# leggedrobotics/qed-splatter

Hardware: AMD Instinct MI355X
Metric: train iters/sec @ 1080p, 500k Gaussians (fwd + loss + bwd + Adam; camera-steps/s over all GPUs) (higher is better)
Workload: dtype f32

## Files before the change

### qed_splatter_amd/csrc/project.hip

```cpp
#include "qed_common.h"

namespace qed {

struct Cam {
    float R[9];
    float t[3];
    float fx, fy, cx, cy;
    float campos[3];
};

__device__ __forceinline__ Cam load_cam(const float* __restrict__ viewmats, const float* __restrict__ Ks, int c) {
    Cam cam;
    const float* V = viewmats + 16 * c;
    const float* K = Ks + 9 * c;
#pragma unroll
    for (int i = 0; i < 3; ++i) {
#pragma unroll
        for (int j = 0; j < 3; ++j) cam.R[3 * i + j] = V[4 * i + j];
        cam.t[i] = V[4 * i + 3];
    }
    cam.fx = K[0]; cam.fy = K[4]; cam.cx = K[2]; cam.cy = K[5];
#pragma unroll
    for (int j = 0; j < 3; ++j)
        cam.campos[j] = campos_component(cam.R[0 + j], cam.R[3 + j], cam.R[6 + j], cam.t[0], cam.t[1], cam.t[2]);
// ... 262 lines not shown
        float mx = 0.f, my = 0.f, z = 0.f, ca = 0.f, cb = 0.f, cc = 0.f, op = 0.f;
        float rgb[3] = {0.f, 0.f, 0.f};
        if (p.valid) {
            rad = (int)p.radius;
            mx = p.mx; my = p.my; z = p.z; ca = p.ca; cb = p.cb; cc = p.cc;
            op = op_raw;
            if (flags & QED_F_LOGIT_OPAC) op = sigmoidf_dev(op);
            if (flags & QED_F_ANTIALIASED) op *= p.comp;
            if (sh_degree >= 0) {
                const float dir[3] = {mean[0] - cam.campos[0], mean[1] - cam.campos[1], mean[2] - cam.campos[2]};
                float J[9];
                unsigned mask;
                sh_color_jac_dyn(sh_degree, sh0 + (size_t)n * sh0_stride, shN + (size_t)n * shN_stride, dir, rgb, J, mask);
                if (sh_jac != nullptr) {
#pragma unroll
                    for (int i = 0; i < 9; ++i) sh_jac[(size_t)i * total + slot] = J[i];
                    sh_jac[(size_t)9 * total + slot] = __uint_as_float(mask);
                }
            } else {
                const float* cptr = sh0 + (size_t)n * sh0_stride;
                rgb[0] = cptr[0]; rgb[1] = cptr[1]; rgb[2] = cptr[2];
                if (flags & QED_F_SIGMOID_COLORS) {
                    rgb[0] = sigmoidf_dev(rgb[0]); rgb[1] = sigmoidf_dev(rgb[1]); rgb[2] = sigmoidf_dev(rgb[2]);
                }
            }
            const float tau = logf(255.f * op);
            int x0, y0, x1, y1;
            if (flags & QED_F_TIGHT_TILES) tight_tile_rect(mx, my, p.radius, ca, cb, cc, tau, tile_w, tile_h, x0, y0, x1, y1);
            else tile_rect(mx, my, p.radius, tile_w, tile_h, x0, y0, x1, y1);
            ntiles = (x1 - x0) * (y1 - y0);
            m_c0 = make_float4(mx, my, ca, cb); m_cc = cc; m_tau = tau; m_rect = pack_tile_rect(x0, y0, x1);
            r0 = make_float4(mx, my, ca, cb);
            r1 = make_float4(cc, op, rgb[0], rgb[1]);
            r2 = make_float4(rgb[2], (flags & QED_F_DEPTH_CHANNEL) ? z : 0.f, tau,
                             __uint_as_float(pack_tile_rect(x0, y0, x1)));
        }
        radii[slot] = rad;
        means2d[2 * slot] = mx; means2d[2 * slot + 1] = my;
        depths[slot] = z;
        conics[3 * slot] = ca; conics[3 * slot + 1] = cb; conics[3 * slot + 2] = cc;
        opac_out[slot] = op;
        colors_out[3 * slot] = rgb[0]; colors_out[3 * slot + 1] = rgb[1]; colors_out[3 * slot + 2] = rgb[2];
        splats[3 * slot] = r0; splats[3 * slot + 1] = r1; splats[3 * slot + 2] = r2;
    }
    if (tile_masks != nullptr) {
        __shared__ __attribute__((aligned(16))) float4 s_c0[4][64];
        __shared__ __attribute__((aligned(16))) float4 s_c1[4][64];
        __shared__ unsigned s_rect[4][64];
        __shared__ int s_pref[4][65];
        __shared__ int s_nz[4][64];
        __shared__ unsigned long long s_start[4][64];
        __shared__ unsigned long long s_mask[4][64];
        const int lane = threadIdx.x & 63, wid = threadIdx.x >> 6;
        const int cand = ntiles <= 64 ? ntiles : 0;
        int x = cand;
#pragma unroll
        for (int o = 1; o < 64; o <<= 1) {
            const int y = __shfl_up(x, o, 64);
            if (lane >= o) x += y;
        }
        const int pref = x - cand;
        const int wtot = __shfl(x, 63, 64);
        const unsigned long long nz = __ballot(cand > 0);
        s_pref[wid][lane] = pref;
        s_c0[wid][lane] = make_float4(m_c0.x, m_c0.y, m_c0.w, m_tau);
        s_c1[wid][lane] = make_float4(0.5f * m_c0.z, 0.5f * m_cc, __builtin_amdgcn_rcpf(m_c0.z), __builtin_amdgcn_rcpf(m_cc));
        s_rect[wid][lane] = m_rect;
        s_mask[wid][lane] = 0ull;
        s_start[wid][lane] = 0ull;
        if (cand > 0) s_nz[wid][__popcll(nz & ((1ull << lane) - 1ull))] = lane;
        __builtin_amdgcn_fence(__ATOMIC_ACQ_REL, "wavefront");
        __builtin_amdgcn_wave_barrier();
        if (cand > 0) atomicOr(&s_start[wid][pref >> 6], 1ull << (pref & 63));
        __builtin_amdgcn_fence(__ATOMIC_ACQ_REL, "wavefront");
        __builtin_amdgcn_wave_barrier();
        int before = 0;
        for (int j0 = 0; j0 < wtot; j0 += 64) {
            const unsigned long long word = s_start[wid][j0 >> 6];
            const int j = j0 + lane;
            const int k = before + __popcll(word & ((2ull << lane) - 1ull)) - 1;
            before += __popcll(word);
            if (j >= wtot) continue;
            const int g = s_nz[wid][k];
            const int local = j - s_pref[wid][g];
            const float4 c0 = s_c0[wid][g], c1 = s_c1[wid][g];
            const unsigned r = s_rect[wid][g];
            const int w = (int)(r >> 22);
            const int row = (int)(((float)local + 0.5f) * __builtin_amdgcn_rcpf((float)w));
            const int tx = (int)(r & 2047u) + local - row * w, ty = (int)((r >> 11) & 2047u) + row;
            CullGauss cg;
            cg.b = c0.z; cg.ha = c1.x; cg.hc = c1.y; cg.ia = c1.z; cg.ic = c1.w;
            cg.X0 = (float)(tx * QED_TILE) + 0.5f - c0.x; cg.Y0 = (float)(ty * QED_TILE) + 0.5f - c0.y;
            const float ax = fmaxf(fabsf(cg.X0), fabsf(cg.X0 + 15.f)), ay = fmaxf(fabsf(cg.Y0), fabsf(cg.Y0 + 15.f));
            cg.thr = c0.w + 1e-3f + 8e-6f * (2.f * (cg.ha * ax * ax + cg.hc * ay * ay) + fabsf(cg.b) * ax * ay);
            if (tile_may_touch(cg)) atomicOr(&s_mask[wid][g], 1ull << local);
        }
        __builtin_amdgcn_fence(__ATOMIC_ACQ_REL, "wavefront");
        __builtin_amdgcn_wave_barrier();
        if (slot < total) {
            unsigned long long mask = ~0ull;
            if (cand > 0) { mask = s_mask[wid][lane]; ntiles = __popcll(mask); }
            reinterpret_cast<uint4*>(tile_masks)[slot] = make_uint4((unsigned)ntiles, m_rect, (unsigned)mask, (unsigned)(mask >> 32));
        }
    }
    if (slot < total) tiles_per_gauss[slot] = ntiles;
    __shared__ int wsum[4];
    const int v = wave_sum_i(ntiles);
    if ((threadIdx.x & 63) == 0) wsum[threadIdx.x >> 6] = v;
    __syncthreads();
    if (threadIdx.x == 0) block_sums[blockIdx.x] = wsum[0] + wsum[1] + wsum[2] + wsum[3];
}

template <int DEG>
__device__ __forceinline__ void sh_bwd(const float* __restrict__ sh0, const float* __restrict__ shN,
                                       const float* dir, const float* v_rgb_in, float* v_coef ,
                                       float* v_dir ) {
    constexpr int K = (DEG + 1) * (DEG + 1);
    const float n2 = dir[0] * dir[0] + dir[1] * dir[1] + dir[2] * dir[2];
    const float inorm = rsqrtf(n2);
    const float x = dir[0] * inorm, y = dir[1] * inorm, z = dir[2] * inorm;
    float b[K];
    sh_basis<DEG>(x, y, z, b);
    float c[3 * K];
    load_sh<K>(sh0, shN, c);
    float col[3] = {0.f, 0.f, 0.f};
#pragma unroll
    for (int k = 0; k < K; ++k) {
        col[0] += b[k] * c[3 * k]; col[1] += b[k] * c[3 * k + 1]; col[2] += b[k] * c[3 * k + 2];
    }
    float v[3];
#pragma unroll
    for (int ch = 0; ch < 3; ++ch) v[ch] = (col[ch] + 0.5f >= 0.f) ? v_rgb_in[ch] : 0.f;
#pragma unroll
    for (int k = 0; k < K; ++k) {
        v_coef[3 * k] += b[k] * v[0]; v_coef[3 * k + 1] += b[k] * v[1]; v_coef[3 * k + 2] += b[k] * v[2];
    }
    if constexpr (DEG > 0) {
        float bx[K], by[K], bz[K];
        sh_basis_grad<DEG>(x, y, z, bx, by, bz);
        float vx = 0.f, vy = 0.f, vz = 0.f;
#pragma unroll
        for (int k = 1; k < K; ++k) {
            const float w = c[3 * k] * v[0] + c[3 * k + 1] * v[1] + c[3 * k + 2] * v[2];
            vx += bx[k] * w; vy += by[k] * w; vz += bz[k] * w;
        }
        const float dot = vx * x + vy * y + vz * z;
        v_dir[0] += (vx - dot * x) * inorm;
        v_dir[1] += (vy - dot * y) * inorm;
        v_dir[2] += (vz - dot * z) * inorm;
    }
}

template <int DEG, bool STREAM>
__device__ __forceinline__ void sh_bwd_jac(const float* __restrict__ jac , size_t plane,
                                           const float* dir, const float* v_rgb_in, float* __restrict__ o0,
                                           float* __restrict__ oN, float* v_coef, float* v_dir , bool compact,
                                           float* stage_b = nullptr ,
                                           float* stage_v = nullptr) {
    constexpr int K = (DEG + 1) * (DEG + 1);
    float J[9];
#pragma unroll
    for (int i = 0; i < (DEG > 0 ? 9 : 0); ++i) J[i] = jac[(size_t)i * plane];
    const unsigned mask = __float_as_uint(jac[(size_t)9 * plane]);
    const float n2 = dir[0] * dir[0] + dir[1] * dir[1] + dir[2] * dir[2];
    const float inorm = rsqrtf(n2);
    const float x = dir[0] * inorm, y = dir[1] * inorm, z = dir[2] * inorm;
    float v[3];
#pragma unroll
    for (int ch = 0; ch < 3; ++ch) v[ch] = (mask >> ch & 1u) ? v_rgb_in[ch] : 0.f;
    if (STREAM && compact) {
        o0[0] = v[0]; o0[1] = v[1]; o0[2] = v[2];
    } else {
        float b[K];
        sh_basis<DEG>(x, y, z, b);
        if constexpr (STREAM) {
            o0[0] = b[0] * v[0]; o0[1] = b[0] * v[1]; o0[2] = b[0] * v[2];
            if (stage_b != nullptr) {
                constexpr int KS = (K + 3) & ~3;
#pragma unroll
                for (int k4 = 0; k4 < KS / 4; ++k4)
                    reinterpret_cast<float4*>(stage_b)[k4] =
                        make_float4(b[4 * k4], 4 * k4 + 1 < K ? b[4 * k4 + 1] : 0.f, 4 * k4 + 2 < K ? b[4 * k4 + 2] : 0.f,
                                    4 * k4 + 3 < K ? b[4 * k4 + 3] : 0.f);
                *reinterpret_cast<float4*>(stage_v) = make_float4(v[0], v[1], v[2], 0.f);
            } else {
#pragma unroll
                for (int k = 1; k < K; ++k) {
                    oN[3 * (k - 1)] = b[k] * v[0]; oN[3 * (k - 1) + 1] = b[k] * v[1]; oN[3 * (k - 1) + 2] = b[k] * v[2];
                }
            }
        } else {
#pragma unroll
            for (int k = 0; k < K; ++k) {
                v_coef[3 * k] += b[k] * v[0]; v_coef[3 * k + 1] += b[k] * v[1]; v_coef[3 * k + 2] += b[k] * v[2];
            }
        }
    }
    if constexpr (DEG > 0) {
        const float vx = J[0] * v[0] + J[1] * v[1] + J[2] * v[2];
        const float vy = J[3] * v[0] + J[4] * v[1] + J[5] * v[2];
        const float vz = J[6] * v[0] + J[7] * v[1] + J[8] * v[2];
        const float dot = vx * x + vy * y + vz * z;
        v_dir[0] += (vx - dot * x) * inorm;
        v_dir[1] += (vy - dot * y) * inorm;
        v_dir[2] += (vz - dot * z) * inorm;
    }
}

template <int DEG>
__device__ __forceinline__ void sh_bwd_stream(const float* __restrict__ sh0, const float* __restrict__ shN,
                                              const float* dir, const float* v_rgb_in, float* __restrict__ o0,
                                              float* __restrict__ oN, float* v_dir , bool compact) {
    constexpr int K = (DEG + 1) * (DEG + 1);
    const float n2 = dir[0] * dir[0] + dir[1] * dir[1] + dir[2] * dir[2];
    const float inorm = rsqrtf(n2);
    const float x = dir[0] * inorm, y = dir[1] * inorm, z = dir[2] * inorm;
    float b[K];
    sh_basis<DEG>(x, y, z, b);
    float col[3] = {0.f, 0.f, 0.f};
    float S[3][3] = {{0.f, 0.f, 0.f}, {0.f, 0.f, 0.f}, {0.f, 0.f, 0.f}};
    {
        float bx[K], by[K], bz[K];
        sh_basis_grad<DEG>(x, y, z, bx, by, bz);
#pragma unroll
        for (int k = 0; k < K; ++k) {
            const float* ck = k == 0 ? sh0 : shN + 3 * (k - 1);
#pragma unroll
            for (int ch = 0; ch < 3; ++ch) {
                const float c = ck[ch];
                col[ch] += b[k] * c;
                if (k > 0) { S[0][ch] += bx[k] * c; S[1][ch] += by[k] * c; S[2][ch] += bz[k] * c; }
            }
        }
    }
    float v[3];
#pragma unroll
    for (int ch = 0; ch < 3; ++ch) v[ch] = (col[ch] + 0.5f >= 0.f) ? v_rgb_in[ch] : 0.f;
    if (compact) {
        o0[0] = v[0]; o0[1] = v[1]; o0[2] = v[2];
    } else {
        o0[0] = b[0] * v[0]; o0[1] = b[0] * v[1]; o0[2] = b[0] * v[2];
#pragma unroll
        for (int k = 1; k < K; ++k) {
            oN[3 * (k - 1)] = b[k] * v[0]; oN[3 * (k - 1) + 1] = b[k] * v[1]; oN[3 * (k - 1) + 2] = b[k] * v[2];
        }
    }
    if constexpr (DEG > 0) {
        const float vx = S[0][0] * v[0] + S[0][1] * v[1] + S[0][2] * v[2];
        const float vy = S[1][0] * v[0] + S[1][1] * v[1] + S[1][2] * v[2];
        const float vz = S[2][0] * v[0] + S[2][1] * v[1] + S[2][2] * v[2];
        const float dot = vx * x + vy * y + vz * z;
        v_dir[0] += (vx - dot * x) * inorm;
        v_dir[1] += (vy - dot * y) * inorm;
        v_dir[2] += (vz - dot * z) * inorm;
    }
}

template <int K>
__device__ __forceinline__ void sh_grad_store_staged(const float* __restrict__ stage ,
                                                     int lane, float* __restrict__ out ,
                                                     int stride, int n_rows) {
    constexpr int KS = (K + 3) & ~3, FP = 3 * (K - 1);
    const float* sv = stage + 64 * KS;
    int g = lane / FP, j = lane - g * FP;
#pragma unroll 5
    for (int it = 0; it < FP; ++it) {
        const int k = (j * 171) >> 9;
        const int ch = j - 3 * k;
        if (g < n_rows) out[(size_t)g * stride + j] = stage[g * KS + k + 1] * sv[4 * g + ch];
        g += 64 / FP; j += 64 % FP;
        if (j >= FP) { j -= FP; ++g; }
    }
}

template <int DEG, bool ONE_CAM, bool JAC = false>
#ifndef QED_PBWD_WAVES
#define QED_PBWD_WAVES 2
#endif
__global__ void __launch_bounds__(256) __attribute__((amdgpu_waves_per_eu(QED_PBWD_WAVES, QED_PBWD_WAVES)))
project_bwd_kernel(int N, int C, const float* __restrict__ means, const float* __restrict__ quats,
                   const float* __restrict__ scales, const float* __restrict__ opacities,
                   const float* __restrict__ sh0, int sh0_stride, const float* __restrict__ shN, int shN_stride,
                   const float* __restrict__ viewmats, const float* __restrict__ Ks, int width, int height,
                   float eps2d, unsigned flags, const int* __restrict__ radii, const float4* __restrict__ vsplat,
                   float* __restrict__ v_means, float* __restrict__ v_quats, float* __restrict__ v_scales,
                   float* __restrict__ v_opacities, float* __restrict__ v_sh0, int v_sh0_stride,
                   float* __restrict__ v_shN, int v_shN_stride, float* __restrict__ v_viewmats,
                   const float* __restrict__ sh_jac) {
    constexpr int K = DEG < 0 ? 1 : (DEG + 1) * (DEG + 1);
    const int n = blockIdx.x * 256 + threadIdx.x;
    const bool active = n < N;

    float vm[3] = {0.f, 0.f, 0.f}, vq[4] = {0.f, 0.f, 0.f, 0.f}, vs[3] = {0.f, 0.f, 0.f}, vo = 0.f;
    constexpr bool kStreamSH = ONE_CAM && DEG >= 0;
    float vcoef[kStreamSH ? 1 : 3 * K];
#pragma unroll
    for (int i = 0; i < (kStreamSH ? 1 : 3 * K); ++i) vcoef[i] = 0.f;
    bool sh_written = false;
    constexpr bool kStageSH = JAC && kStreamSH && K > 1;
    constexpr int kKS = (K + 3) & ~3;
    constexpr int kStageFloats = kStageSH ? 64 * (kKS + 4) : 1;
    __shared__ __attribute__((aligned(16))) float s_stage[4 * kStageFloats];
    float* const stage_wave = s_stage + (threadIdx.x >> 6) * kStageFloats;
    const bool staged = kStageSH && !(flags & QED_F_SH_GRAD_COMPACT);
    float* const stage_b = staged ? stage_wave + (threadIdx.x & 63) * kKS : nullptr;
    float* const stage_v = staged ? stage_wave + 64 * kKS + 4 * (threadIdx.x & 63) : nullptr;

    float mean[3] = {0.f, 0.f, 0.f}, qraw[4] = {1.f, 0.f, 0.f, 0.f}, q[4], sraw[3] = {0.f, 0.f, 0.f}, s[3];
    float qin = 1.f, oraw = 0.f, oact = 0.f;
    if (active) {
        mean[0] = means[3 * n]; mean[1] = means[3 * n + 1]; mean[2] = means[3 * n + 2];
        qraw[0] = quats[4 * n]; qraw[1] = quats[4 * n + 1]; qraw[2] = quats[4 * n + 2]; qraw[3] = quats[4 * n + 3];
        sraw[0] = scales[3 * n]; sraw[1] = scales[3 * n + 1]; sraw[2] = scales[3 * n + 2];
        oraw = opacities[n];
    }
    qin = rsqrtf(qraw[0] * qraw[0] + qraw[1] * qraw[1] + qraw[2] * qraw[2] + qraw[3] * qraw[3]);
#pragma unroll
    for (int i = 0; i < 4; ++i) q[i] = qraw[i] * qin;
#pragma unroll
    for (int i = 0; i < 3; ++i) s[i] = (flags & QED_F_LOG_SCALES) ? __expf(sraw[i]) : sraw[i];
    oact = (flags & QED_F_LOGIT_OPAC) ? sigmoidf_dev(oraw) : oraw;

    for (int c = 0; c < C; ++c) {
        const Cam cam = load_cam(viewmats, Ks, c);
        const size_t slot = (size_t)c * N + n;
        const bool vis = active && radii[slot] > 0;
        float vR[9] = {0.f, 0.f, 0.f, 0.f, 0.f, 0.f, 0.f, 0.f, 0.f}, vt[3] = {0.f, 0.f, 0.f};
        if constexpr (kStageSH) {
            if (staged && !vis) {
#pragma unroll
                for (int k4 = 0; k4 < kKS / 4; ++k4) reinterpret_cast<float4*>(stage_b)[k4] = make_float4(0.f, 0.f, 0.f, 0.f);
                *reinterpret_cast<float4*>(stage_v) = make_float4(0.f, 0.f, 0.f, 0.f);
            }
        }
        if (vis) {
            Proj p;
            project_one(cam, mean, q, s, width, height, eps2d, -3.0e38f, 3.0e38f, -1.f, p);
            const float4 g0 = vsplat[4 * slot], g1 = vsplat[4 * slot + 1], g2 = vsplat[4 * slot + 2];
            const float v_mx = g0.x, v_my = g0.y;
            float v_ca = g1.x, v_cb = g1.y, v_cc = g1.z;
            const float v_op = g1.w;
            const float v_rgb[3] = {g2.x, g2.y, g2.z};
            const float v_depth = (flags & QED_F_DEPTH_CHANNEL) ? g2.w : 0.f;

            float v_comp = 0.f;
            if (flags & QED_F_ANTIALIASED) {
                vo += v_op * p.comp;
                v_comp = v_op * oact;
            } else {
                vo += v_op;
            }
            const float g01 = 0.5f * v_cb;
            const float bh = 0.5f * (p.A + p.Cc), hd = 0.5f * (p.A - p.Cc);
            const float rr = __builtin_amdgcn_sqrtf(hd * hd + p.B * p.B);
            const float lp = bh + rr, ilp = __builtin_amdgcn_rcpf(lp), lm = p.det * ilp, ilm = __builtin_amdgcn_rcpf(lm);
            float ux, uy;
            if (hd >= 0.f) { ux = hd + rr; uy = p.B; }
            else { ux = p.B; uy = rr - hd; }
            const float un = ux * ux + uy * uy;
            if (un > 0.f) { const float ir = __builtin_amdgcn_rsqf(un); ux *= ir; uy *= ir; } else { ux = 1.f; uy = 0.f; }
            const float wx = -uy, wy = ux;
            const float gux = v_ca * ux + g01 * uy, guy = g01 * ux + v_cc * uy;
            const float gwx = v_ca * wx + g01 * wy, gwy = g01 * wx + v_cc * wy;
            float hpp = -(ux * gux + uy * guy) * ilp * ilp;
            float hpm = -(ux * gwx + uy * gwy) * ilp * ilm;
            float hmm = -(wx * gwx + wy * gwy) * ilm * ilm;
            if (flags & QED_F_ANTIALIASED) {
                const float det_conic = 1.f / p.det;
                const float v_sqr = v_comp * 0.5f / (p.comp + 1e-6f);
                const float om = 1.f - p.comp * p.comp;
                hpp += v_sqr * (om * ilp - eps2d * det_conic);
                hmm += v_sqr * (om * ilm - eps2d * det_conic);
            }
            float vT[6];
#pragma unroll
            for (int j = 0; j < 3; ++j) {
                const float pu = ux * p.Tm[j] + uy * p.Tm[3 + j], pw = wx * p.Tm[j] + wy * p.Tm[3 + j];
                const float qu = hpp * pu + hpm * pw, qw = hpm * pu + hmm * pw;
                vT[j] = 2.f * (ux * qu + wx * qw);
                vT[3 + j] = 2.f * (uy * qu + wy * qw);
            }
            const float rz = p.rz, rz2 = rz * rz, rz3 = rz2 * rz;
            const float j00 = cam.fx * rz, j02 = -cam.fx * p.tx * rz2;
            const float j11 = cam.fy * rz, j12 = -cam.fy * p.ty * rz2;
            const float vJ00 = vT[0] * p.W[0] + vT[1] * p.W[1] + vT[2] * p.W[2];
            const float vJ02 = vT[0] * p.W[6] + vT[1] * p.W[7] + vT[2] * p.W[8];
            const float vJ11 = vT[3] * p.W[3] + vT[4] * p.W[4] + vT[5] * p.W[5];
            const float vJ12 = vT[3] * p.W[6] + vT[4] * p.W[7] + vT[5] * p.W[8];
            float vW[9];
#pragma unroll
            for (int j = 0; j < 3; ++j) {
                vW[j] = j00 * vT[j];
                vW[3 + j] = j11 * vT[3 + j];
                vW[6 + j] = j02 * vT[j] + j12 * vT[3 + j];
            }
            float vx = v_mx * cam.fx * rz;
            float vy = v_my * cam.fy * rz;
            float vz = -v_mx * cam.fx * p.x * rz2 - v_my * cam.fy * p.y * rz2 - vJ00 * cam.fx * rz2 -
                       vJ11 * cam.fy * rz2 + v_depth;
            if (!p.clamp_x) {
                vx += -cam.fx * rz2 * vJ02;
                vz += 2.f * cam.fx * p.tx * rz3 * vJ02;
            } else {
                vz += cam.fx * p.tx * rz3 * vJ02;
            }
            if (!p.clamp_y) {
                vy += -cam.fy * rz2 * vJ12;
                vz += 2.f * cam.fy * p.ty * rz3 * vJ12;
            } else {
                vz += cam.fy * p.ty * rz3 * vJ12;
            }
            float vmw[3];
#pragma unroll
            for (int j = 0; j < 3; ++j) vmw[j] = cam.R[j] * vx + cam.R[3 + j] * vy + cam.R[6 + j] * vz;
            float vM[9];
#pragma unroll
            for (int i = 0; i < 3; ++i)
#pragma unroll
                for (int j = 0; j < 3; ++j)
                    vM[3 * i + j] = cam.R[i] * vW[j] + cam.R[3 + i] * vW[3 + j] + cam.R[6 + i] * vW[6 + j];
            float vdir[3] = {0.f, 0.f, 0.f};
            if constexpr (DEG >= 0) {
                const float dir[3] = {mean[0] - cam.campos[0], mean[1] - cam.campos[1], mean[2] - cam.campos[2]};
                if constexpr (JAC) {
                    const size_t plane = (size_t)C * N;
                    sh_bwd_jac<(DEG < 0 ? 0 : DEG), kStreamSH>(sh_jac + slot, plane, dir, v_rgb,
                                                                v_sh0 + (size_t)n * v_sh0_stride,
                                                                v_shN + (size_t)n * v_shN_stride, vcoef, vdir,
                                                                (flags & QED_F_SH_GRAD_COMPACT) != 0, stage_b, stage_v);
                    sh_written = true;
                } else if constexpr (kStreamSH) {
                    sh_bwd_stream<(DEG < 0 ? 0 : DEG)>(sh0 + (size_t)n * sh0_stride, shN + (size_t)n * shN_stride, dir,
                                                       v_rgb, v_sh0 + (size_t)n * v_sh0_stride,
                                                       v_shN + (size_t)n * v_shN_stride, vdir,
                                                       (flags & QED_F_SH_GRAD_COMPACT) != 0);
                    sh_written = true;
                } else {
                    sh_bwd<(DEG < 0 ? 0 : DEG)>(sh0 + (size_t)n * sh0_stride, shN + (size_t)n * shN_stride, dir, v_rgb,
                                                vcoef, vdir);
                }
            } else {
                if (flags & QED_F_SIGMOID_COLORS) {
                    const float* cptr = sh0 + (size_t)n * sh0_stride;
#pragma unroll
                    for (int ch = 0; ch < 3; ++ch) {
                        const float sg = sigmoidf_dev(cptr[ch]);
                        vcoef[ch] += v_rgb[ch] * sg * (1.f - sg);
                    }
                } else {
                    vcoef[0] += v_rgb[0]; vcoef[1] += v_rgb[1]; vcoef[2] += v_rgb[2];
                }
            }
            vm[0] += vmw[0] + vdir[0]; vm[1] += vmw[1] + vdir[1]; vm[2] += vmw[2] + vdir[2];
            float vRq[9];
#pragma unroll
            for (int i = 0; i < 3; ++i)
#pragma unroll
                for (int j = 0; j < 3; ++j) {
                    vRq[3 * i + j] = vM[3 * i + j] * s[j];
                    vs[j] += vM[3 * i + j] * p.Rq[3 * i + j];
                }
            const float w = q[0], x = q[1], y = q[2], z = q[3];
            float vqn[4];
            vqn[0] = 2.f * (x * (vRq[7] - vRq[5]) + y * (vRq[2] - vRq[6]) + z * (vRq[3] - vRq[1]));
            vqn[1] = 2.f * (-2.f * x * (vRq[4] + vRq[8]) + y * (vRq[1] + vRq[3]) + z * (vRq[2] + vRq[6]) +
                            w * (vRq[7] - vRq[5]));
            vqn[2] = 2.f * (x * (vRq[1] + vRq[3]) - 2.f * y * (vRq[0] + vRq[8]) + z * (vRq[5] + vRq[7]) +
                            w * (vRq[2] - vRq[6]));
            vqn[3] = 2.f * (x * (vRq[2] + vRq[6]) + y * (vRq[5] + vRq[7]) - 2.f * z * (vRq[0] + vRq[4]) +
                            w * (vRq[3] - vRq[1]));
            vq[0] += vqn[0]; vq[1] += vqn[1]; vq[2] += vqn[2]; vq[3] += vqn[3];

            if (v_viewmats != nullptr) {
                const float vmc[3] = {vx, vy, vz};
#pragma unroll
                for (int i = 0; i < 3; ++i) {
#pragma unroll
                    for (int j = 0; j < 3; ++j) {
                        vR[3 * i + j] = vmc[i] * mean[j] + vW[3 * i] * p.M[3 * j] + vW[3 * i + 1] * p.M[3 * j + 1] +
                                        vW[3 * i + 2] * p.M[3 * j + 2];
                    }
                    vt[i] = vmc[i];
                }
#pragma unroll
                for (int i = 0; i < 3; ++i) {
                    const float rv = cam.R[3 * i] * vdir[0] + cam.R[3 * i + 1] * vdir[1] + cam.R[3 * i + 2] * vdir[2];
#pragma unroll
                    for (int j = 0; j < 3; ++j) vR[3 * i + j] += rv * cam.campos[j];
                    vt[i] += rv;
                }
            }
        }
        if constexpr (kStageSH) {
            if (staged) {
                __builtin_amdgcn_fence(__ATOMIC_RELEASE, "wavefront");
                __builtin_amdgcn_wave_barrier();
                __builtin_amdgcn_fence(__ATOMIC_ACQUIRE, "wavefront");
                const int n0 = blockIdx.x * 256 + (threadIdx.x & ~63);
                sh_grad_store_staged<K>(stage_wave, threadIdx.x & 63, v_shN + (size_t)n0 * v_shN_stride, v_shN_stride,
                                        N - n0);
            }
        }
        if (v_viewmats != nullptr) {
#pragma unroll
            for (int i = 0; i < 12; ++i) {
                float v = i < 9 ? vR[i] : vt[i - 9];
                v = wave_sum(v);
                if ((threadIdx.x & 63) == 0 && v != 0.f) {
                    const int row = i < 9 ? i / 3 : i - 9, col = i < 9 ? i % 3 : 3;
                    atomicAdd(&v_viewmats[16 * c + 4 * row + col], v);
                }
            }
        }
    }
    if (!active) return;
    const float dq = vq[0] * q[0] + vq[1] * q[1] + vq[2] * q[2] + vq[3] * q[3];
#pragma unroll
    for (int i = 0; i < 4; ++i) v_quats[4 * n + i] = (vq[i] - dq * q[i]) * qin;
#pragma unroll
    for (int i = 0; i < 3; ++i) {
        v_means[3 * n + i] = vm[i];
        v_scales[3 * n + i] = (flags & QED_F_LOG_SCALES) ? vs[i] * s[i] : vs[i];
    }
    v_opacities[n] = (flags & QED_F_LOGIT_OPAC) ? vo * oact * (1.f - oact) : vo;
    float* o0 = v_sh0 + (size_t)n * v_sh0_stride;
    if constexpr (kStreamSH) {
        if (!sh_written) {
            o0[0] = 0.f; o0[1] = 0.f; o0[2] = 0.f;
            if (K > 1 && !(flags & QED_F_SH_GRAD_COMPACT) && !staged) {
                float* oN = v_shN + (size_t)n * v_shN_stride;
#pragma unroll
                for (int i = 0; i < 3 * (K - 1); ++i) oN[i] = 0.f;
            }
        }
    } else {
        o0[0] = vcoef[0]; o0[1] = vcoef[1]; o0[2] = vcoef[2];
        if constexpr (K > 1) {
            float* oN = v_shN + (size_t)n * v_shN_stride;
#pragma unroll
            for (int i = 0; i < 3 * (K - 1); ++i) oN[i] = vcoef[3 + i];
        }
    }
}

template <int DEG>
__global__ void __launch_bounds__(256)
sh_grad_from_views_kernel(int N, int n_views, const float* __restrict__ means, const float* __restrict__ viewmats,
                          long long viewmat_stride, const float* __restrict__ v_views, long long view_stride,
                          float scale, float* __restrict__ v_sh0, int v_sh0_stride, float* __restrict__ v_shN,
                          int v_shN_stride) {
    constexpr int K = (DEG + 1) * (DEG + 1);
    const int n = blockIdx.x * 256 + threadIdx.x;
    if (n >= N) return;
    const float mean[3] = {means[3 * n], means[3 * n + 1], means[3 * n + 2]};
    float acc[3 * K];
#pragma unroll
    for (int i = 0; i < 3 * K; ++i) acc[i] = 0.f;
    for (int c = 0; c < n_views; ++c) {
        const float* vm = viewmats + viewmat_stride * c;
        const float* vv = v_views + view_stride * c + (size_t)n * 3;
        const float v[3] = {vv[0], vv[1], vv[2]};
        if (v[0] == 0.f && v[1] == 0.f && v[2] == 0.f) continue;
        float dir[3];
#pragma unroll
        for (int j = 0; j < 3; ++j)
            dir[j] = mean[j] - campos_component(vm[0 + j], vm[4 + j], vm[8 + j], vm[3], vm[7], vm[11]);
        const float inorm = rsqrtf(dir[0] * dir[0] + dir[1] * dir[1] + dir[2] * dir[2]);
        float b[K];
        sh_basis<DEG>(dir[0] * inorm, dir[1] * inorm, dir[2] * inorm, b);
#pragma unroll
        for (int k = 0; k < K; ++k) {
            acc[3 * k] += b[k] * v[0]; acc[3 * k + 1] += b[k] * v[1]; acc[3 * k + 2] += b[k] * v[2];
        }
    }
    float* o0 = v_sh0 + (size_t)n * v_sh0_stride;
    o0[0] = acc[0] * scale; o0[1] = acc[1] * scale; o0[2] = acc[2] * scale;
    if constexpr (K > 1) {
        float* oN = v_shN + (size_t)n * v_shN_stride;
#pragma unroll
        for (int i = 0; i < 3 * (K - 1); ++i) oN[i] = acc[3 + i] * scale;
    }
}

__global__ void camera_setup_kernel(int C, const float* __restrict__ c2w, const float* __restrict__ intr,
                                    float* __restrict__ viewmats, float* __restrict__ Ks) {
    const int c = blockIdx.x * blockDim.x + threadIdx.x;
    if (c >= C) return;
    const float* m = c2w + 12 * c;
    float R[9], t[3];
#pragma unroll
    for (int i = 0; i < 3; ++i) {
        R[3 * i] = m[4 * i];
        R[3 * i + 1] = -m[4 * i + 1];
        R[3 * i + 2] = -m[4 * i + 2];
        t[i] = m[4 * i + 3];
    }
    float* V = viewmats + 16 * c;
#pragma unroll
    for (int i = 0; i < 3; ++i) {
#pragma unroll
        for (int j = 0; j < 3; ++j) V[4 * i + j] = R[3 * j + i];
        V[4 * i + 3] = -(R[i] * t[0] + R[3 + i] * t[1] + R[6 + i] * t[2]);
    }
    V[12] = 0.f; V[13] = 0.f; V[14] = 0.f; V[15] = 1.f;
    float* K = Ks + 9 * c;
    K[0] = intr[4 * c]; K[1] = 0.f; K[2] = intr[4 * c + 2];
    K[3] = 0.f; K[4] = intr[4 * c + 1]; K[5] = intr[4 * c + 3];
    K[6] = 0.f; K[7] = 0.f; K[8] = 1.f;
}

}

using namespace qed;

extern "C" int qed_camera_setup(int32_t C, const float* c2w, const float* intrinsics, float* viewmats, float* Ks,
                                void* stream) {
    QED_REQUIRE(C >= 1 && c2w && intrinsics && viewmats && Ks, "bad arguments");
    hipLaunchKernelGGL(camera_setup_kernel, dim3((C + 63) / 64), dim3(64), 0, (hipStream_t)stream, C, c2w, intrinsics,
                       viewmats, Ks);
    return check_launch("qed_camera_setup");
}

extern "C" int qed_project_fwd(int32_t N, int32_t C, const float* means, const float* quats, const float* scales,
                               const float* opacities, const float* sh0, int32_t sh0_stride, const float* shN,
                               int32_t shN_stride, int32_t sh_degree, const float* viewmats, const float* Ks,
                               int32_t width, int32_t height, int32_t tile_w, int32_t tile_h, float eps2d,
                               float near_plane, float far_plane, float radius_clip, uint32_t flags, int32_t* radii,
                               float* means2d, float* depths, float* conics, float* opac_out, float* colors_out,
                               float* splats, int32_t* tiles_per_gauss, uint64_t* tile_masks, int32_t* block_sums,
                               float* viewmats_out, float* Ks_out, float* sh_jac, void* stream) {
    QED_REQUIRE(N >= 0 && C >= 1, "N >= 0 and C >= 1 required");
    QED_REQUIRE(sh_degree <= 3, "SH degree > 3 unsupported (reference config uses sh_degree = 3)");
    QED_REQUIRE(width > 0 && height > 0 && tile_w > 0 && tile_h > 0, "bad image / tile extents");
    QED_REQUIRE((long long)tile_w * tile_h < (1ll << 30), "too many tiles");
    if (N == 0) return QED_OK;
    QED_REQUIRE(means && quats && scales && opacities && sh0 && viewmats && Ks, "null input");
    QED_REQUIRE(sh_degree <= 0 || shN, "shN required for sh_degree > 0");
    QED_REQUIRE(radii && means2d && depths && conics && opac_out && colors_out && splats && tiles_per_gauss &&
                    block_sums, "null output");
    QED_REQUIRE(!(flags & QED_F_CAMERA_C2W) || (viewmats_out && Ks_out), "QED_F_CAMERA_C2W needs viewmats_out and Ks_out");
    QED_REQUIRE(tile_masks == nullptr || (flags & QED_F_TIGHT_TILES), "tile_masks goes with QED_F_TIGHT_TILES");
    QED_REQUIRE(((uintptr_t)tile_masks & 15) == 0, "tile_masks must be 16-byte aligned");
    const long long total = (long long)C * N;
    const unsigned grid = (unsigned)((total + 255) / 256);
#define QED_LAUNCH_PF(ONE)                                                                                           \
    hipLaunchKernelGGL(project_fwd_kernel<ONE>, dim3(grid), dim3(256), 0, (hipStream_t)stream, N, C, means, quats,   \
                       scales, opacities, sh0, sh0_stride, shN, shN_stride, sh_degree, viewmats, Ks, width, height,  \
                       tile_w, tile_h, eps2d, near_plane, far_plane, radius_clip, flags, radii, means2d, depths,     \
                       conics, opac_out, colors_out, (float4*)splats, tiles_per_gauss, block_sums, viewmats_out, Ks_out,    \
                       sh_degree >= 0 ? sh_jac : nullptr, (unsigned long long*)tile_masks)
    if (C == 1) QED_LAUNCH_PF(true);
    else QED_LAUNCH_PF(false);
#undef QED_LAUNCH_PF
    return check_launch("qed_project_fwd");
}

extern "C" int qed_project_bwd(int32_t N, int32_t C, const float* means, const float* quats, const float* scales,
                               const float* opacities, const float* sh0, int32_t sh0_stride, const float* shN,
                               int32_t shN_stride, int32_t sh_degree, const float* viewmats, const float* Ks,
                               int32_t width, int32_t height, float eps2d, uint32_t flags, const int32_t* radii,
                               const float* vsplat, float* v_means, float* v_quats, float* v_scales,
                               float* v_opacities, float* v_sh0, int32_t v_sh0_stride, float* v_shN,
                               int32_t v_shN_stride, float* v_viewmats, const float* sh_jac, void* stream) {
    QED_REQUIRE(N >= 0 && C >= 1, "N >= 0 and C >= 1 required");
// ... 80 lines not shown
```

### qed_splatter_amd/csrc/ssim.hip

```cpp
#include "qed_common.h"

namespace qed {

constexpr int kWin = 11;
constexpr int kHalo = kWin - 1;

__device__ __constant__ float c_win[kWin] = {
    1.028380357e-03f, 7.598758209e-03f, 3.600077331e-02f, 1.093606874e-01f, 2.130055279e-01f, 2.660117149e-01f,
    2.130055279e-01f, 1.093606874e-01f, 3.600077331e-02f, 7.598758209e-03f, 1.028380357e-03f};

template <int TW_, int TH_, int NT_ = 256>
struct SsimTile {
    static constexpr int TW = TW_, TH = TH_, NT = NT_;
    static constexpr int NW = NT / 64;
    static constexpr int PW = TW + kHalo, PH = TH + kHalo;
    static constexpr int SP = TW + 12;
    static constexpr int SH = TW + 4;
    static constexpr int ROW_ITEMS = PH * (TW / 4);
    static constexpr bool WAVE_COLUMNS = PH <= 64;
    static constexpr int ROW_SLOTS = WAVE_COLUMNS ? 64 * (TW / 4) : ROW_ITEMS;
    static __device__ __forceinline__ bool row_item(int i, int& gx, int& py) {
        if constexpr (WAVE_COLUMNS) { gx = i >> 6; py = i & 63; return py < PH; }
        else { gx = i / PH; py = i - gx * PH; return true; }
    }
// ... 171 lines not shown
#pragma unroll
            for (int o = 0; o < CB; ++o) {
                float a = 0.f;
#pragma unroll
                for (int d = 0; d < kWin; ++d) a += w[d] * v[o + d];
                st[q][o] = a;
            }
        }
        const int qx = ox + tx;
        float* m = maps + (size_t)k * 3 * n_out;
#pragma unroll
        for (int o = 0; o < CB; ++o) {
            const int qy = oy + ty0 + o;
            if (qx < Wo && qy < Ho) {
                const float mu1 = st[0][o], mu2 = st[1][o];
                const float mm = mu1 * mu1 + mu2 * mu2;
                const float var12 = st[2][o] - mm, cov = st[3][o] - mu1 * mu2;
                const float a1 = 2.f * mu1 * mu2 + C1, b1 = mm + C1;
                const float a2 = 2.f * cov + C2, b2 = var12 + C2;
                const float ib1 = __builtin_amdgcn_rcpf(b1), ib2 = __builtin_amdgcn_rcpf(b2);
                const float lum = a1 * ib1, cs = a2 * ib2;
                acc += lum * cs;
                const float dS_dmu1 = cs * (2.f * mu2 * ib1 - a1 * ib1 * ib1 * 2.f * mu1);
                const float dS_dvar1 = -lum * a2 * ib2 * ib2;
                const float dS_dcov = lum * 2.f * ib2;
                if (maps != nullptr) {
                    const size_t q = (size_t)qy * Wo + qx;
                    m[q] = dS_dmu1 - 2.f * mu1 * dS_dvar1 - mu2 * dS_dcov;
                    m[n_out + q] = dS_dvar1;
                    m[2 * n_out + q] = dS_dcov;
                }
            }
        }
    }
    acc = wave_sum(acc);
    if ((tid & 63) == 0) s_red[tid >> 6] = acc;
    __syncthreads();
    if (tid == 0) {
        float tot = 0.f;
#pragma unroll
        for (int q = 0; q < T::NW; ++q) tot += s_red[q];
        ssim_sum[block_id] = tot;
    }
}

struct LossFuse {
    const float* depth;
    const float* gt_depth;
    float* sums;
    int n_loss_blocks;
    float w_rgb;
    float depth_lambda;
    const float* g_main;
    const float* g_depth;
    float* v_render;
    float* v_alpha;
    float* v_depth;
    float4* zero_buf;
    long long zero_vec;
};

template <bool COMPOSITE, bool MASKED, class T, int FUSE = 0>
#ifndef QED_SSIM_BWD_WAVES
#define QED_SSIM_BWD_WAVES 4
#endif
#ifndef QED_SSIM_FUSED_WAVES
#define QED_SSIM_FUSED_WAVES 3
#endif
__global__ void __launch_bounds__(T::NT)
__attribute__((amdgpu_waves_per_eu(FUSE >= 3 ? QED_SSIM_FUSED_WAVES : QED_SSIM_BWD_WAVES,
                                   FUSE >= 3 ? QED_SSIM_FUSED_WAVES : QED_SSIM_BWD_WAVES)))
ssim_bwd_kernel(int H, int W, int channels, const float* __restrict__ pred, const float* __restrict__ alpha,
                const float* __restrict__ bg, const float* __restrict__ gt, const float* __restrict__ mask,
                const float* __restrict__ maps, float scale, const float* __restrict__ scale_dev,
                float* __restrict__ v_pred, LossFuse lf) {
    static_assert(FUSE == 0 || (FUSE == 1 && !COMPOSITE) || ((FUSE == 3 || FUSE == 4) && COMPOSITE), "see LossFuse");
    constexpr int TW = T::TW, PW = T::PW, PH = T::PH, SP = T::SP, SH = T::SH, CB = T::CB;
    __shared__ __attribute__((aligned(16))) float s_m[3][PH * SP];
    __shared__ __attribute__((aligned(16))) float s_h[3][PH * SH];
    __shared__ float s_red[2][T::NW];
    const int Ho = H - kHalo, Wo = W - kHalo;
    const int nbx = (W + TW - 1) / TW;
    const int blk = xcd_remap(blockIdx.x, gridDim.x);
    const int by = blk / nbx, bx = blk - by * nbx;
    const int ox = bx * TW, oy = by * T::TH;
    const int tid = threadIdx.x;
    const size_t n_out = (size_t)Ho * Wo;
    float w[kWin];
#pragma unroll
    for (int d = 0; d < kWin; ++d) w[d] = c_win[d];
    const int spy = tid / PW, spx = tid - spy * PW;
    const bool stager = tid < T::RPP * PW;
    const int tx = tid % TW, ty0 = (tid / TW) * CB;
    const int ix = ox + tx;
    if (scale_dev != nullptr) scale *= scale_dev[0];
    float l1 = 0.f, dsum = 0.f, w_rgb = 0.f, w_d = 0.f, dmax = 0.f;
    float ep_d[CB], ep_a[CB], ep_gd[CB];
    bool inside[CB];
#pragma unroll
    for (int o = 0; o < CB; ++o) { ep_d[o] = 0.f; ep_a[o] = 1.f; ep_gd[o] = 0.f; inside[o] = ix < W && oy + ty0 + o < H; }
    if constexpr (FUSE != 0) {
        w_rgb = lf.w_rgb;
        if constexpr (FUSE == 1) w_rgb *= lf.g_main != nullptr ? lf.g_main[0] : 0.f;
        const bool want_depth = FUSE == 4 || (FUSE == 1 && lf.v_depth != nullptr);
        float ep_nv[4] = {0.f, 0.f, 0.f, 0.f}, ep_dm[4] = {-3.0e38f, -3.0e38f, -3.0e38f, -3.0e38f};
        if constexpr (FUSE == 4) {
            static_assert(kLossMaxGrid <= 4 * T::NT, "four partials per thread cover pass 1's grid");
#pragma unroll
            for (int j = 0; j < 4; ++j) {
                const int b = tid + T::NT * j;
                const int bc = b < lf.n_loss_blocks ? b : 0;
                const float nv = loss_part(lf.sums, 0)[bc], dm = loss_part(lf.sums, 1)[bc];
                ep_nv[j] = b < lf.n_loss_blocks ? nv : 0.f;
                ep_dm[j] = b < lf.n_loss_blocks ? dm : -3.0e38f;
            }
        }
        if (want_depth) {
#pragma unroll
            for (int o = 0; o < CB; ++o) {
                const size_t pix = (size_t)min(oy + ty0 + o, H - 1) * W + min(ix, W - 1);
                if constexpr (FUSE == 4) { ep_d[o] = pred[4 * pix + 3]; ep_a[o] = alpha[pix]; }
                else ep_d[o] = lf.depth[pix];
                ep_gd[o] = lf.gt_depth[pix];
            }
        }
        if constexpr (FUSE == 4) {
            float nv = (ep_nv[0] + ep_nv[1]) + (ep_nv[2] + ep_nv[3]);
            float dm = fmaxf(fmaxf(ep_dm[0], ep_dm[1]), fmaxf(ep_dm[2], ep_dm[3]));
            nv = wave_sum(nv);
            dm = wave_max(dm);
            if ((tid & 63) == 0) { s_red[0][tid >> 6] = nv; s_red[1][tid >> 6] = dm; }
            __syncthreads();
            float nvalid = 0.f;
            dmax = -3.0e38f;
#pragma unroll
            for (int q = 0; q < T::NW; ++q) { nvalid += s_red[0][q]; dmax = fmaxf(dmax, s_red[1][q]); }
            w_d = nvalid > 0.f ? lf.depth_lambda / nvalid : 0.f;
        } else if constexpr (FUSE == 1) {
            const float nvalid = lf.sums[2];
            w_d = nvalid > 0.f ? (lf.g_depth != nullptr ? lf.g_depth[0] : 0.f) * lf.depth_lambda / nvalid : 0.f;
        }
    }
    if constexpr (FUSE != 0) {
        if (lf.zero_buf != nullptr) {
            const long long per = (lf.zero_vec + gridDim.x - 1) / gridDim.x;
            const long long lo = (long long)blockIdx.x * per, hi = lo + per < lf.zero_vec ? lo + per : lf.zero_vec;
            for (long long i = lo + tid; i < hi; i += T::NT) lf.zero_buf[i] = make_float4(0.f, 0.f, 0.f, 0.f);
        }
    }
    float r0[CB], r1[CB];
    float mo[CB];
#pragma unroll
    for (int o = 0; o < CB; ++o) mo[o] = MASKED ? mask[(size_t)min(oy + ty0 + o, H - 1) * W + min(ix, W - 1)] : 1.f;
#pragma unroll 1
    for (int k = 0; k < 3; ++k) {
        const float* m = maps + (size_t)k * 3 * n_out;
        float mv[T::LOADS][3];
#pragma unroll
        for (int j = 0; j < T::LOADS; ++j) {
            const int qy = oy + spy + T::RPP * j - kHalo, qx = ox + spx - kHalo;
            const size_t q = (size_t)min(max(qy, 0), Ho - 1) * Wo + min(max(qx, 0), Wo - 1);
            const float al = m[q], bl = m[n_out + q], cl = m[2 * n_out + q];
            const bool in = qy >= 0 && qy < Ho && qx >= 0 && qx < Wo;
            mv[j][0] = in ? al : 0.f; mv[j][1] = in ? bl : 0.f; mv[j][2] = in ? cl : 0.f;
        }
        float xo[CB], yo[CB], pre[CB];
        const float bgk = COMPOSITE ? bg[k] : 0.f;
#pragma unroll
        for (int o = 0; o < CB; ++o) {
            const size_t pix = (size_t)min(oy + ty0 + o, H - 1) * W + min(ix, W - 1);
            if constexpr (COMPOSITE) {
                pre[o] = pred[pix * channels + k] + (1.f - alpha[pix]) * bgk;
                xo[o] = fminf(fmaxf(pre[o], 0.f), 1.f);
            } else {
                pre[o] = 0.f;
                xo[o] = pred[pix * 3 + k];
            }
            yo[o] = gt[pix * 3 + k];
            if constexpr (MASKED) { xo[o] *= mo[o]; yo[o] *= mo[o]; }
        }
        __syncthreads();
        if (stager) {
#pragma unroll
            for (int j = 0; j < T::LOADS; ++j)
                if (spy + T::RPP * j < PH) {
#pragma unroll
                    for (int q = 0; q < 3; ++q) s_m[q][(spy + T::RPP * j) * SP + spx] = mv[j][q];
                }
        }
        __syncthreads();
        for (int i = tid; i < T::ROW_SLOTS; i += T::NT) {
            int gx, py;
            if (!T::row_item(i, gx, py)) continue;
            const int o = py * SH + 4 * gx;
#pragma unroll
            for (int q = 0; q < 3; ++q) {
                float v[16];
                read16(&s_m[q][py * SP + 4 * gx], v);
                *reinterpret_cast<float4*>(&s_h[q][o]) = window4(v, w);
            }
        }
        __syncthreads();
        float g[3][CB];
#pragma unroll
        for (int q = 0; q < 3; ++q) {
            float v[CB + kHalo];
#pragma unroll
            for (int j = 0; j < CB + kHalo; ++j) v[j] = s_h[q][(ty0 + j) * SH + tx];
#pragma unroll
            for (int o = 0; o < CB; ++o) {
                float a = 0.f;
#pragma unroll
                for (int d = 0; d < kWin; ++d) a += w[d] * v[o + d];
                g[q][o] = a;
            }
        }
#pragma unroll
        for (int o = 0; o < CB; ++o) {
            float r = scale * (g[0][o] + 2.f * xo[o] * g[1][o] + yo[o] * g[2][o]);
            if constexpr (MASKED) r *= mo[o];
            if constexpr (FUSE != 0) {
                const float diff = xo[o] - yo[o];
                if (inside[o]) l1 += fabsf(diff);
                const float sg = diff > 0.f ? 1.f : (diff < 0.f ? -1.f : 0.f);
                r = w_rgb * sg * mo[o] + r;
                if constexpr (COMPOSITE)
                    r = (pre[o] >= 0.f && pre[o] <= 1.f) ? r : 0.f;
            }
            if (k == 0) r0[o] = r;
            else if (k == 1) r1[o] = r;
            else if (inside[o]) {
                const size_t pix = (size_t)(oy + ty0 + o) * W + ix;
                if constexpr (FUSE == 0 || FUSE == 1) {
                    Float3 v; v.a = r0[o]; v.b = r1[o]; v.c = r;
                    *reinterpret_cast<Float3*>(v_pred + pix * 3) = v;
                    if constexpr (FUSE == 1) {
                        if (lf.v_depth != nullptr) {
                            const float dp = ep_d[o] * mo[o], dg = ep_gd[o] * mo[o];
                            float gd = 0.f;
                            if (isfinite(dp) && isfinite(dg) && dg > 0.f) {
                                const float dd = dp - dg;
                                gd = w_d * (dd > 0.f ? 1.f : (dd < 0.f ? -1.f : 0.f)) * mo[o];
                            }
                            lf.v_depth[pix] = gd;
                        }
                    }
                } else if constexpr (FUSE == 4) {
                    const float a = ep_a[o];
                    const float dg = ep_gd[o] * mo[o];
                    const float dp = (a > 0.f ? ep_d[o] : dmax) * mo[o];
                    float v3 = 0.f;
                    if (isfinite(dp) && isfinite(dg) && dg > 0.f) {
                        const float dd = dp - dg;
                        dsum += fabsf(dd);
                        if (a > 0.f) v3 = w_d * (dd > 0.f ? 1.f : (dd < 0.f ? -1.f : 0.f)) * mo[o];
                    }
                    *reinterpret_cast<float4*>(lf.v_render + 4 * pix) = make_float4(r0[o], r1[o], r, v3);
                    lf.v_alpha[pix] = -((r0[o] * bg[0] + r1[o] * bg[1]) + r * bgk);
                } else {
                    Float3 v; v.a = r0[o]; v.b = r1[o]; v.c = r;
                    *reinterpret_cast<Float3*>(lf.v_render + 3 * pix) = v;
                    lf.v_alpha[pix] = -((r0[o] * bg[0] + r1[o] * bg[1]) + r * bgk);
                }
            }
        }
    }
    if constexpr (FUSE >= 3) {
        l1 = wave_sum(l1);
        dsum = wave_sum(dsum);
        __syncthreads();
        if ((tid & 63) == 0) { s_red[0][tid >> 6] = l1; s_red[1][tid >> 6] = dsum; }
        __syncthreads();
        if (tid == 0) {
            const int slot = (int)(blockIdx.x % (unsigned)lf.n_loss_blocks);
            float t0 = 0.f, t1 = 0.f;
#pragma unroll
            for (int q = 0; q < T::NW; ++q) { t0 += s_red[0][q]; t1 += s_red[1][q]; }
            atomicAdd(&loss_part(lf.sums, 2)[slot], t0);
            atomicAdd(&loss_part(lf.sums, 3)[slot], t1);
        }
    }
}

#ifndef QED_SSIM_FWD_TW
#define QED_SSIM_FWD_TW 32
#define QED_SSIM_FWD_TH 32
#endif
#ifndef QED_SSIM_FWD_NT
#define QED_SSIM_FWD_NT 256
#endif
#ifndef QED_SSIM_BWD_NT
#define QED_SSIM_BWD_NT 256
#endif
#ifndef QED_SSIM_BWD_TW
#define QED_SSIM_BWD_TW 32
#define QED_SSIM_BWD_TH 32
#endif
using Tile = SsimTile<QED_SSIM_FWD_TW, QED_SSIM_FWD_TH, QED_SSIM_FWD_NT>;
using TileB = SsimTile<QED_SSIM_BWD_TW, QED_SSIM_BWD_TH, QED_SSIM_BWD_NT>;

}

using namespace qed;


extern "C" int64_t qed_ssim_sum_floats(int32_t height, int32_t width) {
    if (height <= kHalo || width <= kHalo) return QED_E_INVALID_ARG;
    return (int64_t)((width - kHalo + Tile::TW - 1) / Tile::TW) * ((height - kHalo + Tile::TH - 1) / Tile::TH);
}

extern "C" int64_t qed_ssim_maps_floats(int32_t height, int32_t width) {
    if (height <= kHalo || width <= kHalo) return QED_E_INVALID_ARG;
    return 9ll * (height - kHalo) * (width - kHalo);
}

static int ssim_fwd_launch(int32_t height, int32_t width, int32_t channels, const float* pred, const float* alpha,
                           const float* background, const float* gt_rgb, const float* mask, float* maps,
                           float* ssim_sum, const TileOrderJob& job, const LossReduceJob& rjob, void* stream,
                           const char* who) {
    QED_REQUIRE(height > kHalo && width > kHalo, "image smaller than the 11 x 11 SSIM window");
    QED_REQUIRE(pred && gt_rgb && ssim_sum, "null buffers");
    QED_REQUIRE(alpha == nullptr || (background && (channels == 3 || channels == 4)), "composite mode needs a background");
    hipStream_t st = (hipStream_t)stream;
    const dim3 grid(((width - kHalo + Tile::TW - 1) / Tile::TW) * ((height - kHalo + Tile::TH - 1) / Tile::TH) +
                    (job.cost4 != nullptr ? 1 : 0) + rjob.n_blocks);
#define QED_SSIM_FWD(COMP, MASK, CHN)                                                                               \
    hipLaunchKernelGGL((ssim_fwd_kernel<COMP, MASK, Tile>), grid, dim3(Tile::NT), 0, st, height, width, CHN, pred, alpha,   \
                       background, gt_rgb, mask, maps, ssim_sum, job, rjob)
    if (alpha != nullptr) { if (mask) QED_SSIM_FWD(true, true, channels); else QED_SSIM_FWD(true, false, channels); }
    else { if (mask) QED_SSIM_FWD(false, true, 3); else QED_SSIM_FWD(false, false, 3); }
#undef QED_SSIM_FWD
// ... 110 lines not shown
```

Before: 1140.

## Hoist and pin per-Gaussian loads, block-reduce viewmat grads, preload SSIM pixels

In the projection backward kernel, all per-Gaussian and per-camera inputs (radii, vsplat gradients, SH Jacobian planes) are issued up front. Empty asm constraints pin them in registers so their latency overlaps with setup math. Viewmat gradient atomics are now reduced across the four waves through shared memory, with one atomic per element per block instead of one per wave. In the SSIM backward kernel, pred/gt/alpha values for all output rows are loaded once as vector loads before the channel loop rather than reloaded per channel. These changes trade extra register pressure and a new __syncthreads for fewer memory round trips and atomics.

```diff
diff --git a/qed_splatter_amd/csrc/project.hip b/qed_splatter_amd/csrc/project.hip
--- a/qed_splatter_amd/csrc/project.hip
+++ b/qed_splatter_amd/csrc/project.hip
@@ -438,16 +438,12 @@
 }
 
 template <int DEG, bool STREAM>
-__device__ __forceinline__ void sh_bwd_jac(const float* __restrict__ jac , size_t plane,
-                                           const float* dir, const float* v_rgb_in, float* __restrict__ o0,
-                                           float* __restrict__ oN, float* v_coef, float* v_dir , bool compact,
+__device__ __forceinline__ void sh_bwd_jac(const float (&J)[9], float mask_bits, const float* dir,
+                                           const float* v_rgb_in, float* __restrict__ o0, float* __restrict__ oN, float* v_coef, float* v_dir , bool compact,
                                            float* stage_b = nullptr ,
                                            float* stage_v = nullptr) {
     constexpr int K = (DEG + 1) * (DEG + 1);
-    float J[9];
-#pragma unroll
-    for (int i = 0; i < (DEG > 0 ? 9 : 0); ++i) J[i] = jac[(size_t)i * plane];
-    const unsigned mask = __float_as_uint(jac[(size_t)9 * plane]);
+    const unsigned mask = __float_as_uint(mask_bits);
     const float n2 = dir[0] * dir[0] + dir[1] * dir[1] + dir[2] * dir[2];
     const float inorm = rsqrtf(n2);
     const float x = dir[0] * inorm, y = dir[1] * inorm, z = dir[2] * inorm;
@@ -558,6 +554,36 @@
         if (j >= FP) { j -= FP; ++g; }
     }
 }
+
+template <bool JAC, bool DEG_POS>
+struct PbwdLoads {
+    int rad;
+    float4 g0, g1, g2;
+    float J[9], mask_bits;
+    __device__ __forceinline__ void load(const int* __restrict__ radii, const float4* __restrict__ vsplat,
+                                         const float* __restrict__ sh_jac, size_t slot, size_t plane) {
+        rad = radii[slot];
+        load_rest(vsplat, sh_jac, slot, plane);
+    }
+    __device__ __forceinline__ void load_rest(const float4* __restrict__ vsplat, const float* __restrict__ sh_jac,
+                                              size_t slot, size_t plane) {
+        g0 = vsplat[4 * slot]; g1 = vsplat[4 * slot + 1]; g2 = vsplat[4 * slot + 2];
+#pragma unroll
+        for (int i = 0; i < 9; ++i) J[i] = (JAC && DEG_POS) ? sh_jac[(size_t)i * plane + slot] : 0.f;
+        mask_bits = JAC ? sh_jac[(size_t)9 * plane + slot] : 0.f;
+    }
+    __device__ __forceinline__ void pin() {
+        asm volatile("" : "+v"(rad), "+v"(g0.x), "+v"(g0.y), "+v"(g0.z), "+v"(g0.w), "+v"(g1.x), "+v"(g1.y), "+v"(g1.z),
+                          "+v"(g1.w), "+v"(g2.x), "+v"(g2.y), "+v"(g2.z), "+v"(g2.w));
+        if constexpr (JAC) {
+            if constexpr (DEG_POS)
+                asm volatile("" : "+v"(J[0]), "+v"(J[1]), "+v"(J[2]), "+v"(J[3]), "+v"(J[4]), "+v"(J[5]), "+v"(J[6]),
+                                  "+v"(J[7]), "+v"(J[8]), "+v"(mask_bits));
+            else
+                asm volatile("" : "+v"(mask_bits));
+        }
+    }
+};
 
 template <int DEG, bool ONE_CAM, bool JAC = false>
 #ifndef QED_PBWD_WAVES
@@ -588,18 +614,25 @@
     constexpr int kStageFloats = kStageSH ? 64 * (kKS + 4) : 1;
     __shared__ __attribute__((aligned(16))) float s_stage[4 * kStageFloats];
     float* const stage_wave = s_stage + (threadIdx.x >> 6) * kStageFloats;
+    __shared__ float s_vm[2][4][12];
     const bool staged = kStageSH && !(flags & QED_F_SH_GRAD_COMPACT);
     float* const stage_b = staged ? stage_wave + (threadIdx.x & 63) * kKS : nullptr;
     float* const stage_v = staged ? stage_wave + 64 * kKS + 4 * (threadIdx.x & 63) : nullptr;
 
-    float mean[3] = {0.f, 0.f, 0.f}, qraw[4] = {1.f, 0.f, 0.f, 0.f}, q[4], sraw[3] = {0.f, 0.f, 0.f}, s[3];
-    float qin = 1.f, oraw = 0.f, oact = 0.f;
-    if (active) {
-        mean[0] = means[3 * n]; mean[1] = means[3 * n + 1]; mean[2] = means[3 * n + 2];
-        qraw[0] = quats[4 * n]; qraw[1] = quats[4 * n + 1]; qraw[2] = quats[4 * n + 2]; qraw[3] = quats[4 * n + 3];
-        sraw[0] = scales[3 * n]; sraw[1] = scales[3 * n + 1]; sraw[2] = scales[3 * n + 2];
-        oraw = opacities[n];
-    }
+    const int nc = active ? n : 0;
+    const size_t plane = (size_t)C * N;
+    float mean[3] = {means[3 * nc], means[3 * nc + 1], means[3 * nc + 2]};
+    float qraw[4] = {quats[4 * nc], quats[4 * nc + 1], quats[4 * nc + 2], quats[4 * nc + 3]};
+    float sraw[3] = {scales[3 * nc], scales[3 * nc + 1], scales[3 * nc + 2]};
+    float oraw = opacities[nc];
+    constexpr bool kPin = DEG <= 1 || (JAC && (ONE_CAM || DEG == 2));
+    PbwdLoads<JAC, (DEG > 0)> ld;
+    if constexpr (ONE_CAM && kPin) ld.load(radii, vsplat, sh_jac, (size_t)nc, plane);
+    if constexpr (kPin)
+        asm volatile("" : "+v"(mean[0]), "+v"(mean[1]), "+v"(mean[2]), "+v"(qraw[0]), "+v"(qraw[1]), "+v"(qraw[2]),
+                          "+v"(qraw[3]), "+v"(sraw[0]), "+v"(sraw[1]), "+v"(sraw[2]), "+v"(oraw));
+    if constexpr (ONE_CAM && kPin) ld.pin();
+    float q[4], s[3], qin, oact;
     qin = rsqrtf(qraw[0] * qraw[0] + qraw[1] * qraw[1] + qraw[2] * qraw[2] + qraw[3] * qraw[3]);
 #pragma unroll
     for (int i = 0; i < 4; ++i) q[i] = qraw[i] * qin;
@@ -609,8 +642,12 @@
 
     for (int c = 0; c < C; ++c) {
         const Cam cam = load_cam(viewmats, Ks, c);
-        const size_t slot = (size_t)c * N + n;
-        const bool vis = active && radii[slot] > 0;
+        if constexpr (!ONE_CAM && kPin) {
+            ld.load(radii, vsplat, sh_jac, (size_t)c * N + nc, plane);
+            ld.pin();
+        }
+        if constexpr (!kPin) ld.rad = active ? radii[(size_t)c * N + n] : 0;
+        const bool vis = active && ld.rad > 0;
         float vR[9] = {0.f, 0.f, 0.f, 0.f, 0.f, 0.f, 0.f, 0.f, 0.f}, vt[3] = {0.f, 0.f, 0.f};
         if constexpr (kStageSH) {
             if (staged && !vis) {
@@ -622,7 +659,8 @@
         if (vis) {
             Proj p;
             project_one(cam, mean, q, s, width, height, eps2d, -3.0e38f, 3.0e38f, -1.f, p);
-            const float4 g0 = vsplat[4 * slot], g1 = vsplat[4 * slot + 1], g2 = vsplat[4 * slot + 2];
+            if constexpr (!kPin) ld.load_rest(vsplat, sh_jac, (size_t)c * N + n, plane);
+            const float4 g0 = ld.g0, g1 = ld.g1, g2 = ld.g2;
             const float v_mx = g0.x, v_my = g0.y;
             float v_ca = g1.x, v_cb = g1.y, v_cc = g1.z;
             const float v_op = g1.w;
@@ -709,8 +747,7 @@
             if constexpr (DEG >= 0) {
                 const float dir[3] = {mean[0] - cam.campos[0], mean[1] - cam.campos[1], mean[2] - cam.campos[2]};
                 if constexpr (JAC) {
-                    const size_t plane = (size_t)C * N;
-                    sh_bwd_jac<(DEG < 0 ? 0 : DEG), kStreamSH>(sh_jac + slot, plane, dir, v_rgb,
+                    sh_bwd_jac<(DEG < 0 ? 0 : DEG), kStreamSH>(ld.J, ld.mask_bits, dir, v_rgb,
                                                                 v_sh0 + (size_t)n * v_sh0_stride,
                                                                 v_shN + (size_t)n * v_shN_stride, vcoef, vdir,
                                                                 (flags & QED_F_SH_GRAD_COMPACT) != 0, stage_b, stage_v);
@@ -788,14 +825,18 @@
             }
         }
         if (v_viewmats != nullptr) {
+            float (*part)[12] = s_vm[c & 1];
 #pragma unroll
             for (int i = 0; i < 12; ++i) {
-                float v = i < 9 ? vR[i] : vt[i - 9];
-                v = wave_sum(v);
-                if ((threadIdx.x & 63) == 0 && v != 0.f) {
-                    const int row = i < 9 ? i / 3 : i - 9, col = i < 9 ? i % 3 : 3;
-                    atomicAdd(&v_viewmats[16 * c + 4 * row + col], v);
-                }
+                const float v = wave_sum(i < 9 ? vR[i] : vt[i - 9]);
+                if ((threadIdx.x & 63) == 0) part[threadIdx.x >> 6][i] = v;
+            }
+            __syncthreads();
+            if (threadIdx.x < 12) {
+                const int i = threadIdx.x;
+                const float v = (part[0][i] + part[1][i]) + (part[2][i] + part[3][i]);
+                const int row = i < 9 ? i / 3 : i - 9, col = i < 9 ? i % 3 : 3;
+                if (v != 0.f) atomicAdd(&v_viewmats[16 * c + 4 * row + col], v);
             }
         }
     }
diff --git a/qed_splatter_amd/csrc/ssim.hip b/qed_splatter_amd/csrc/ssim.hip
--- a/qed_splatter_amd/csrc/ssim.hip
+++ b/qed_splatter_amd/csrc/ssim.hip
@@ -347,6 +347,25 @@
     float mo[CB];
 #pragma unroll
     for (int o = 0; o < CB; ++o) mo[o] = MASKED ? mask[(size_t)min(oy + ty0 + o, H - 1) * W + min(ix, W - 1)] : 1.f;
+    constexpr bool kPreload = FUSE != 1;
+    float pc[CB][3], gc[CB][3], ac[CB];
+    if constexpr (kPreload) {
+        const bool four = FUSE == 4 || (FUSE != 3 && COMPOSITE && channels == 4);
+#pragma unroll
+        for (int o = 0; o < CB; ++o) {
+            const size_t pix = (size_t)min(oy + ty0 + o, H - 1) * W + min(ix, W - 1);
+            const Float3 gv = *reinterpret_cast<const Float3*>(gt + pix * 3);
+            gc[o][0] = gv.a; gc[o][1] = gv.b; gc[o][2] = gv.c;
+            if (four) {
+                const float4 pv = *reinterpret_cast<const float4*>(pred + pix * 4);
+                pc[o][0] = pv.x; pc[o][1] = pv.y; pc[o][2] = pv.z;
+            } else {
+                const Float3 pv = *reinterpret_cast<const Float3*>(pred + pix * 3);
+                pc[o][0] = pv.a; pc[o][1] = pv.b; pc[o][2] = pv.c;
+            }
+            ac[o] = COMPOSITE ? alpha[pix] : 1.f;
+        }
+    }
 #pragma unroll 1
     for (int k = 0; k < 3; ++k) {
         const float* m = maps + (size_t)k * 3 * n_out;
@@ -363,15 +382,25 @@
         const float bgk = COMPOSITE ? bg[k] : 0.f;
 #pragma unroll
         for (int o = 0; o < CB; ++o) {
-            const size_t pix = (size_t)min(oy + ty0 + o, H - 1) * W + min(ix, W - 1);
+            float pk, gk, ak;
+            if constexpr (kPreload) {
+                pk = k == 0 ? pc[o][0] : (k == 1 ? pc[o][1] : pc[o][2]);
+                gk = k == 0 ? gc[o][0] : (k == 1 ? gc[o][1] : gc[o][2]);
+                ak = ac[o];
+            } else {
+                const size_t pix = (size_t)min(oy + ty0 + o, H - 1) * W + min(ix, W - 1);
+                pk = pred[pix * (COMPOSITE ? channels : 3) + k];
+                gk = gt[pix * 3 + k];
+                ak = COMPOSITE ? alpha[pix] : 1.f;
+            }
             if constexpr (COMPOSITE) {
-                pre[o] = pred[pix * channels + k] + (1.f - alpha[pix]) * bgk;
+                pre[o] = pk + (1.f - ak) * bgk;
                 xo[o] = fminf(fmaxf(pre[o], 0.f), 1.f);
             } else {
                 pre[o] = 0.f;
-                xo[o] = pred[pix * 3 + k];
-            }
-            yo[o] = gt[pix * 3 + k];
+                xo[o] = pk;
+            }
+            yo[o] = gk;
             if constexpr (MASKED) { xo[o] *= mo[o]; yo[o] *= mo[o]; }
         }
         __syncthreads();
```

Result: faster. 1154, median of 6 (+1.2%).
